# sec-bit/ckb-zkp

Measured on AMD Instinct MI355X. Metric: Groth16 proofs/sec (2^20 constraints, BN256), higher is better.
Workload: dtype u32 limbs (256-bit Montgomery integers); 1 GPU; Groth16 prove, MiMC-chain R1CS, 1048570 constraints (domain 2^20), 1258284 aux, bn254, G1 x4 + G2 x1 MSM + 4 NTT (7 in the reference: evaluation-form key); curve=bn254, log_domain=20, parallelism=independent proofs x1

## Files before the change

ckb_zkp_amd/csrc/msm.hip:

```cpp
#include <algorithm>
#include <cstdlib>
#include <cstring>
#include <map>
#include <type_traits>
#include <memory>
#include <mutex>
#include <vector>

#include "field_dev.hpp"
#include "internal.hpp"
#include "msm_digits.hpp"
#include "msm_small.hpp"
#include "msm_vtbl.hpp"

namespace zkp {

#if defined(ZKP_NO_SORT_PRIO)
#define ZKP_SORT_PRIO() do { } while (0)
#else
#define ZKP_SORT_PRIO() __builtin_amdgcn_s_setprio(3)
#endif

const MsmVtbl* msm_vtbl_c01();
const MsmVtbl* msm_vtbl_c02();
// ... 820 lines not shown
          constexpr int NT = decltype(nt)::value;
          hipLaunchKernelGGL((sort_hist_kernel<FrP, NT>), dim3(nblocks), dim3(NT), 0, st, sc, n, offset, scan_inf, mont, c, W, wide, nb_w,
                             LB, nbins1, hist, nblocks, tile, lgk);
        };
        if (nt_hist >= 1024) hist_l(std::integral_constant<int, 1024>{});
        else if (nt_hist >= 512) hist_l(std::integral_constant<int, 512>{});
        else hist_l(std::integral_constant<int, 256>{});
        exclusive_scan_u32(st, hist, offs, hist_n, ws.scan_tmp);
        if (staged_sub) {
          auto scat_l = [&](auto nt) {
            constexpr int NT = decltype(nt)::value;
            hipLaunchKernelGGL((sort_scatter_staged_kernel<FrP, NT>), dim3(nblocks), dim3(NT), staged_lds, st, sc, n, offset,
                               scan_inf, mont, be->n, c, W, wide, nb_w, LB, nbins1, offs, nblocks, tile, kv, lgk, grp, staged_sub);
          };
          if (nt_scat >= 1024) scat_l(std::integral_constant<int, 1024>{});
          else if (nt_scat >= 512) scat_l(std::integral_constant<int, 512>{});
          else scat_l(std::integral_constant<int, 256>{});
        } else {
          hipLaunchKernelGGL(sort_scatter_kernel<FrP>, dim3(nblocks), dim3(256), 0, st, sc, n, offset, scan_inf, mont, be->n, c, W, wide,
                             nb_w, LB, nbins1, offs, nblocks, tile, kv, lgk, grp);
        }
      };
      if (be->curve == ZKP_BN254) level1(Bn254Fr{});
      else level1(Bls381Fr{});
    }
    if (timed_scan) {
      ZKP_HIP(hipEventRecord(ctx->ev3, st));
      ZKP_HIP(hipEventSynchronize(ctx->ev3));
      ZKP_HIP(hipEventElapsedTime(ms_scan, ctx->ev2, ctx->ev3));
    }
    if (!reuse && !l1_reuse) ZKP_HIP(hipEventRecord(ws.l1_done, st));
    if (!reuse && !l1_reuse) ctx->mark(st, ":l1");
    if (!reuse)
      hipLaunchKernelGGL(sort_bin_kernel, dim3(nbins1), dim3(SORT_BIN_THREADS), ((size_t)4 << LB) + 4 * (size_t)SORT_BIN_STAGE, st,
                         kv, offs, nblocks, LB, vals, start, end, (l1_reuse || grp) ? be->filter_bit : -1);
    uint32_t* const sorted_vals = vals;
    const uint32_t max_tasks = nb + (uint32_t)(E / be->cap) + 1;
    uint32_t* sched = sw.sched.as<uint32_t>((size_t)2 * (nb + 2) + (size_t)8 * max_tasks + TM_WORDS + 8);
    uint32_t* tcount = sched;
    uint32_t* toff = tcount + (nb + 2);
    uint32_t* task_start = toff + (nb + 2);
    uint32_t* task_len = task_start + max_tasks;
    uint32_t* task_dst = task_len + max_tasks;
    uint32_t* long_list = task_dst + max_tasks;
    uint32_t* tmeta = long_list + max_tasks;
    uint4* desc = reinterpret_cast<uint4*>((reinterpret_cast<uintptr_t>(tmeta + TM_WORDS) + 15) & ~(uintptr_t)15);
    if (!reuse) {
      ZKP_HIP(hipMemsetAsync(tmeta, 0, TM_WORDS * 4, st));
      hipLaunchKernelGGL(task_count_kernel, dim3((nb + 256) / 256), dim3(256), 0, st, start, end, nb, tcount, be->cap);
      exclusive_scan_u32(st, tcount, toff, (size_t)nb + 1, ws.scan_tmp2);
      static const uint32_t tnt = [] { const char* e = getenv("ZKP_TASK_NT"); const int v = e ? atoi(e) : 1024; return (uint32_t)(v >= 1024 ? 1024 : v >= 512 ? 512 : 256); }();
      hipLaunchKernelGGL(task_fill_kernel, dim3((nb + tnt - 1) / tnt), dim3(tnt), 0, st, start, end, toff, nb, task_start,
                         task_len, task_dst, long_list, tmeta, be->cap);
      hipLaunchKernelGGL(task_cursor_kernel, dim3(1), dim3(64), 0, st, tmeta);
      hipLaunchKernelGGL(task_order_kernel, dim3((max_tasks + tnt - 1) / tnt), dim3(tnt), 0, st, task_start, task_len, task_dst,
                         toff + nb, tmeta, desc);
      ZKP_HIP(hipEventRecord(ws.sorted, st));
      ctx->mark(st, ":sorted");
    }
    MsmWorkspace& bws = bucket_ws >= 0 ? ctx->cur->ws[bucket_ws] : ws;
    char* buckets = reinterpret_cast<char*>(bws.buckets.get((size_t)2 * nb * XB + XB));
    char* task_partial = reinterpret_cast<char*>(ws.partial.get((size_t)max_tasks * XB));
    static const bool zero_all = getenv("ZKP_MEMSET_BUCKETS") && atoi(getenv("ZKP_MEMSET_BUCKETS")) != 0;
    const uint32_t init = into >= 0 ? 1u : 0u;
    if (init) {
      ZKP_REQUIRE(bws.chain_nb == nb && bws.chain_xb == XB, ZKP_ERR_BAD_ARG);
      ZKP_HIP(hipStreamWaitEvent(st, bws.acc_done, 0));
    } else if (zero_all) ZKP_HIP(hipMemsetAsync(buckets, 0, (size_t)nb * XB, st));
    else hipLaunchKernelGGL(zero_empty_buckets_kernel, dim3((nb + 255) / 256), dim3(256), 0, st, start, end, nb, buckets, (uint32_t)XB);
    bws.chain_nb = 0;
    const bool timed = ms_accumulate && ctx->profiling;
    if (timed) ZKP_HIP(hipEventRecord(ctx->ev2, st));
    static const uint32_t force_redo = getenv("ZKP_DEBUG_FORCE_REDO") && atoi(getenv("ZKP_DEBUG_FORCE_REDO")) != 0 ? 2u : 0u;
    ctx->mark(st, ":acc0");
    vt->accumulate(st, be->table, sorted_vals, desc, toff + nb, max_tasks, buckets, task_partial,
                   ws.redo.as<uint32_t>((size_t)max_tasks + 1), init | force_redo);
    ctx->mark(st, ":acc1");
    if (timed) {
      ZKP_HIP(hipEventRecord(ctx->ev3, st));
      ZKP_HIP(hipEventSynchronize(ctx->ev3));
      ZKP_HIP(hipEventElapsedTime(ms_accumulate, ctx->ev2, ctx->ev3));
    }
    static const int dbg = [] { const char* e = getenv("ZKP_DEBUG_MSM"); return e ? atoi(e) : 0; }();
    if (dbg) {
      uint32_t* rep = ws.redo.as<uint32_t>((size_t)max_tasks + 1);
      ZKP_HIP(hipStreamSynchronize(st));
      ZKP_HIP(hipMemsetAsync(rep, 0, 32, st));
      hipLaunchKernelGGL(sched_check_kernel, dim3(256), dim3(256), 0, st, toff, long_list, tmeta, nb, max_tasks, rep);
      uint32_t h[8];
      ZKP_HIP(hipMemcpyAsync(h, rep, 32, hipMemcpyDeviceToHost, st));
      ZKP_HIP(hipStreamSynchronize(st));
      printf("[msm] group=%d n=%zu nb=%u max_tasks=%u: toff inversions=%u max tasks/bucket=%u bad long_list=%u n_long=%u n_tasks=%u overflow=%u\n",
             be->group, n, nb, max_tasks, h[0], h[1], h[2], h[3], h[4], h[5]);
      fflush(stdout);
    }
#ifdef ZKP_ABLATION
    if (dbg != 2)
#endif
      vt->combine(st, long_list, tmeta + TM_NLONG, toff, task_partial, buckets, init);
    if (dbg) {
      hipError_t e = hipStreamSynchronize(st);
      printf("[msm] combine: %s\n", hipGetErrorString(e));
      fflush(stdout);
    }
    if (n_entries) {
      *n_entries = E;
      if (ctx->profiling) {
        uint32_t emitted = 0;
        ZKP_HIP(hipMemcpyAsync(&emitted, offs + hist_n - 1, 4, hipMemcpyDeviceToHost, st));
        ZKP_HIP(hipStreamSynchronize(st));
        *n_entries = emitted;
      }
    }
    if (var) {
      VarPlan& vp = var_plan(ctx, c, K, st);
      uint32_t lvl_off = 0, cnt = nb;
      for (int l = 0; l < c - 1; l++) {
        vt->pair(st, buckets + (size_t)lvl_off * XB, buckets + (size_t)(lvl_off + cnt) * XB, cnt / 2);
        lvl_off += cnt;
        cnt /= 2;
      }
      const char* roots = buckets + (size_t)lvl_off * XB;
      char* partial = reinterpret_cast<char*>(ws.tmp.get(((size_t)vp.n1 + 256 + 8) * XB));
      char* R = partial + (size_t)vp.n1 * XB;
      vt->segsum_desc(st, buckets, vp.d1.as<SegDesc>(vp.n1), vp.n1, partial);
      vt->segsum_desc(st, partial, vp.d2.as<SegDesc>(256), 256, R);
      vt->final_var(st, R, roots, c, K, (char*)out_dev_xyzz, out_jac);
      ZKP_HIP(hipGetLastError());
      if (out_xyz_host) {
        ZKP_HIP(hipMemcpyAsync(out_xyz_host, out_jac, jac_words * 4, hipMemcpyDeviceToHost, st));
        ZKP_HIP(hipStreamSynchronize(st));
      }
      return;
    }
    if (defer) {
      bws.chain_nb = nb;
      bws.chain_xb = XB;
      ZKP_HIP(hipEventRecord(bws.acc_done, st));
      vt->write_identity(st, (char*)out_dev_xyzz, out_jac);
      ZKP_HIP(hipGetLastError());
      ZKP_REQUIRE(!out_xyz_host, ZKP_ERR_BAD_ARG);
      return;
    }
#ifdef ZKP_ABLATION
    if (ctx->dbg_skip_k8) return;
#endif
    const int L = c - 1;
    SegPlan plan{};
    plan.L = L;
    const uint32_t chunk = ctx->batch_mode ? SEG_CHUNK_BATCH : SEG_CHUNK;
    plan.chunk = chunk;
    uint32_t lvl_off = 0, cnt = nb, blocks = 0;
    static const bool fuse_seg = !(getenv("ZKP_PAIR_TOP_FUSE_SEG") && atoi(getenv("ZKP_PAIR_TOP_FUSE_SEG")) == 0);
    int l_top = -1;
    char* top_base = nullptr;
    uint32_t top_cnt = 0;
    for (int l = 0; l < L; l++) {
      uint32_t next_off = lvl_off + cnt;
      static const bool top_fused = !(getenv("ZKP_PAIR_TOP") && atoi(getenv("ZKP_PAIR_TOP")) == 0);
      static const uint32_t top_max = [] {
        const char* e = getenv("ZKP_PAIR_TOP_MAX");
        uint32_t v = e ? (uint32_t)atoi(e) : PAIR_TOP_MAX;
        if (v < 2) v = PAIR_TOP_MAX;
        while (v & (v - 1)) v &= v - 1;
        return v;
      }();
      if (!top_fused || cnt > top_max) vt->pair(st, buckets + (size_t)lvl_off * XB, buckets + (size_t)next_off * XB, cnt / 2);
      else if (cnt == top_max || l == 0) {
        if (fuse_seg && cnt / 2 <= chunk) {
          l_top = l;
          top_base = buckets + (size_t)lvl_off * XB;
          top_cnt = cnt;
        } else {
          vt->pair_top(st, buckets + (size_t)lvl_off * XB, cnt);
        }
      }
      plan.first_block[l] = blocks;
      plan.off[l] = lvl_off + 1;
      plan.stride[l] = 2;
      plan.count[l] = cnt / 2;
      blocks += (cnt / 2 + chunk - 1) / chunk;
      lvl_off = next_off;
      cnt /= 2;
    }
    plan.first_block[L] = blocks;
    const char* root = buckets + (size_t)lvl_off * XB;
    char* partial = reinterpret_cast<char*>(ws.tmp.get(((size_t)blocks + 64) * XB));
    char* Obuf = partial + (size_t)blocks * XB;
    if (L > 0 && l_top >= 0) {
      SegPlan low = plan;
      low.L = l_top;
      const uint32_t blocks_low = plan.first_block[l_top];
      vt->pair_top_segsum(st, top_base, top_cnt, buckets, &low, partial, blocks_low);
      SegPlan p2{};
      p2.L = L;
      p2.chunk = chunk;
      for (int l = 0; l < L; l++) {
        p2.first_block[l] = l;
        if (l < l_top) {
          p2.off[l] = plan.first_block[l];
          p2.stride[l] = 1;
          p2.count[l] = plan.first_block[l + 1] - plan.first_block[l];
        } else {
          p2.off[l] = plan.off[l];
          p2.stride[l] = plan.stride[l];
          p2.count[l] = plan.count[l];
        }
        ZKP_REQUIRE(p2.count[l] <= chunk, ZKP_ERR_BAD_ARG);
      }
      p2.first_block[L] = L;
      vt->segsum(st, partial, &p2, Obuf, L, buckets, l_top);
    } else if (L > 0) {
      vt->segsum(st, buckets, &plan, partial, blocks, nullptr, 1 << 30);
      SegPlan p2{};
      p2.L = L;
      p2.chunk = chunk;
      for (int l = 0; l < L; l++) {
        p2.first_block[l] = l;
        p2.off[l] = plan.first_block[l];
        p2.stride[l] = 1;
        p2.count[l] = plan.first_block[l + 1] - plan.first_block[l];
        ZKP_REQUIRE(p2.count[l] <= chunk, ZKP_ERR_BAD_ARG);
      }
      p2.first_block[L] = L;
      vt->segsum(st, partial, &p2, Obuf, L, nullptr, 1 << 30);
    }
    vt->final(st, Obuf, L, root, (char*)out_dev_xyzz, out_jac);
    ctx->mark(st, ":reduced");
  }
  ZKP_HIP(hipGetLastError());
  if (out_xyz_host) {
    ZKP_HIP(hipMemcpyAsync(out_xyz_host, out_jac, jac_words * 4, hipMemcpyDeviceToHost, st));
    ZKP_HIP(hipStreamSynchronize(st));
  }
}

void msm_run_multi(zkp_ctx* ctx, size_t count, const uint64_t* handles, const size_t* offsets,
                   const uint64_t* const* scalars_dev, const size_t* ns, bool montgomery, uint64_t* out_xyz_host,
                   size_t slot_words) {
  if (count == 0) return;
  const size_t jw = slot_words;
  zkp_lane* L = ctx->cur;
  if (ctx->pinned_cap < count * jw * 4) {
    if (ctx->pinned) (void)hipHostFree(ctx->pinned);
    ctx->pinned = nullptr;
    ctx->pinned_cap = 0;
    ZKP_HIP(hipHostMalloc(reinterpret_cast<void**>(&ctx->pinned), count * jw * 4 + 4096));
    ctx->pinned_cap = count * jw * 4 + 4096;
  }
  constexpr int NW = zkp_lane::N_WS_MSM;
  const int NL = std::max(1, std::min(ctx->cfg.msm_batch_lanes, (int)zkp_ctx::N_LANES));
  auto stream_of = [&](int li, int w) { return w == 0 ? ctx->lanes[li].stream : ctx->lanes[li].ws[w].stream; };
  struct Restore {
    zkp_ctx* c;
    zkp_lane* cur;
    int idx;
    ~Restore() {
      c->cur = cur;
      c->cur_idx = idx;
    }
  } restore{ctx, ctx->cur, ctx->cur_idx};
  ZKP_HIP(hipEventRecord(L->ev_fork, L->stream));
  for (int li = 0; li < NL; li++)
    for (int w = 0; w < NW; w++)
      if (stream_of(li, w) != L->stream) ZKP_HIP(hipStreamWaitEvent(stream_of(li, w), L->ev_fork, 0));
  for (size_t k = 0; k < count; k++) {
    const int li = (int)((k / NW) % NL), w = (int)(k % NW);
    auto be = get_bases(ctx, handles[k]);
    const size_t words = 3 * (size_t)be->vt->fN;
    ZKP_REQUIRE(words <= jw, ZKP_ERR_BAD_ARG);
    ZKP_REQUIRE(offsets[k] <= be->n, ZKP_ERR_BAD_ARG);
    const size_t n = std::min(ns[k], be->n - offsets[k]);
    ctx->cur = &ctx->lanes[li];
    ctx->cur_idx = li;
    msm_run(ctx, handles[k], offsets[k], scalars_dev[k], n, montgomery, nullptr, nullptr, nullptr, nullptr, w);
    ZKP_HIP(hipMemcpyAsync(ctx->pinned + k * jw, ctx->lanes[li].ws[w].out.p, words * 4, hipMemcpyDeviceToHost, stream_of(li, w)));
  }
  ctx->cur = restore.cur;
  ctx->cur_idx = restore.idx;
  for (int li = 0; li < NL; li++)
    for (int w = 0; w < NW; w++) {
      if (stream_of(li, w) == L->stream) continue;
      ZKP_HIP(hipEventRecord(ctx->lanes[li].ws[w].done, stream_of(li, w)));
      ZKP_HIP(hipStreamWaitEvent(L->stream, ctx->lanes[li].ws[w].done, 0));
    }
  ZKP_HIP(hipStreamSynchronize(L->stream));
  memcpy(out_xyz_host, ctx->pinned, count * jw * 4);
}

void msm_run_batch(zkp_ctx* ctx, uint64_t handle, size_t count, const size_t* offsets, const uint64_t* const* scalars_dev,
                   const size_t* ns, bool montgomery, uint64_t* out_xyz_host) {
  if (count == 0) return;
  std::vector<uint64_t> handles(count, handle);
  msm_run_multi(ctx, count, handles.data(), offsets, scalars_dev, ns, montgomery, out_xyz_host,
                3 * (size_t)get_bases(ctx, handle)->vt->fN);
}

void msm_var_run(zkp_ctx* ctx, int curve, int group, const uint64_t* xy_host, const uint8_t* inf_host,
                 const uint64_t* scalars_host, size_t n, bool montgomery, uint64_t* out_xyz_host) {
  BasesEntry e;
  e.curve = curve;
  e.group = group;
  e.vt = msm_vtbl(curve, group);
  e.n = n;
  e.var = true;
  e.owns = false;
  e.c = n >= 4096 ? 16 : 8;
  if (const char* env = getenv("ZKP_MSM_VAR_C")) {
    int c = atoi(env);
    if (c == 4 || c == 8 || c == 16) e.c = c;
  }
  e.W = 256 / e.c;
  e.wide = e.W;
  while ((1 << e.lgk) < e.W) e.lgk++;
  ZKP_REQUIRE((double)n * e.W < 2147483000.0, ZKP_ERR_BAD_ARG);
  hipStream_t st = ctx->cur->stream;
  const size_t ab = e.vt->aff_bytes;
  uint64_t* sdev = nullptr;
  if (n) {
// ... 221 lines not shown
```

ckb_zkp_amd/csrc/msm_group.hip:

```cpp
#include "bucket_dev.hpp"
#include "coop_dev.hpp"
#include "ec_dev.hpp"
#include "glv.hpp"
#include "msm_vtbl.hpp"

#ifndef ZKP_CFG_CURVE
#error "compile with -DZKP_CFG_CURVE=0|1 -DZKP_CFG_GROUP=1|2"
#endif

namespace zkp {

#if ZKP_CFG_CURVE == 0
using CfgFq = Bn254Fq;
using CfgFr = Bn254Fr;
constexpr int CFG_BITS = 254;
#else
using CfgFq = Bls381Fq;
using CfgFr = Bls381Fr;
constexpr int CFG_BITS = 255;
#endif
#if ZKP_CFG_GROUP == 1
using CfgF = Fp<CfgFq>;
#else
using CfgF = Fp2<CfgFq>;
#endif
#define ZKP_CAT3(a, b, c) a##b##c
#define ZKP_SYM(name, cu, gr) ZKP_CAT3(name, cu, gr)
#define ZKP_CFG_SYM(name) ZKP_SYM(name##_c, ZKP_CFG_CURVE, ZKP_CFG_GROUP)

namespace ZKP_CFG_SYM(cfg) {}
using namespace ZKP_CFG_SYM(cfg);

template <class F>
__global__ void ingest_kernel(char* table, const uint8_t* inf, size_t n) {
  size_t i = (size_t)blockIdx.x * blockDim.x + threadIdx.x;
  if (i >= n) return;
  if (inf && inf[i]) Affine<F>::inf().store(table + i * Affine<F>::BYTES);
}

template <class F>
__global__ __launch_bounds__(128) void precompute_kernel(char* table, size_t n, int c, int W, int wide) {
  size_t i = (size_t)blockIdx.x * blockDim.x + threadIdx.x;
  if (i >= n) return;
  Affine<F> p = Affine<F>::load(table + i * Affine<F>::BYTES);
  XYZZ<F> acc = XYZZ<F>::from_affine(p);
  for (int w = 1; w < W; w++) {
    const int cw = w - 1 < wide ? c : c - 1;
    for (int k = 0; k < cw; k++) acc = acc.dbl();
    Affine<F> a = acc.to_affine();
    a.store(table + ((size_t)w * n + i) * Affine<F>::BYTES);
    acc = XYZZ<F>::from_affine(a);
  }
}

template <class F>
__global__ __launch_bounds__(256) void pair_kernel(const char* __restrict__ in, char* __restrict__ out,
                                                   uint32_t count) {
  __builtin_amdgcn_s_setprio(3);
  uint32_t k = blockIdx.x * blockDim.x + threadIdx.x;
  if (k >= count) return;
  BkPoint<F>::add_mem(in + (size_t)(2 * k) * BkPoint<F>::BYTES, in + (size_t)(2 * k + 1) * BkPoint<F>::BYTES,
                      out + (size_t)k * BkPoint<F>::BYTES);
}

constexpr int PAIR_TOP_THREADS = 512;
template <class F>
__device__ __forceinline__ void pair_top_body(char* __restrict__ base, uint32_t cnt) {
  char* in = base;
  for (; cnt > 1; cnt >>= 1) {
    char* out = in + (size_t)cnt * BkPoint<F>::BYTES;
    bool coop = false;
    if constexpr (QuadCoop<F>::ON) coop = cnt / 2 <= PAIR_TOP_THREADS / 4;
    if constexpr (QuadCoop<F>::ON) {
      if (coop) {
        const uint32_t k = threadIdx.x >> 2;
        if (k < cnt / 2)
          quad_add_any<F>(in + (size_t)(2 * k) * BkPoint<F>::BYTES, in + (size_t)(2 * k + 1) * BkPoint<F>::BYTES,
                          out + (size_t)k * BkPoint<F>::BYTES, threadIdx.x & 3);
      }
    }
    if (!coop)
      for (uint32_t k = threadIdx.x; k < cnt / 2; k += PAIR_TOP_THREADS)
        BkPoint<F>::add_mem(in + (size_t)(2 * k) * BkPoint<F>::BYTES, in + (size_t)(2 * k + 1) * BkPoint<F>::BYTES,
                            out + (size_t)k * BkPoint<F>::BYTES);
    __threadfence_block();
    __syncthreads();
    in = out;
  }
}
template <class F>
__global__ __launch_bounds__(PAIR_TOP_THREADS) void pair_top_kernel(char* __restrict__ base, uint32_t cnt) {
  __builtin_amdgcn_s_setprio(3);
  pair_top_body<F>(base, cnt);
}

template <class F>
__device__ __forceinline__ void segsum_body(const char* __restrict__ base, const SegPlan& plan, char* __restrict__ partial, uint32_t block,
                                            const char* __restrict__ base_hi, int l_hi) {
  extern __shared__ __attribute__((aligned(16))) char smem[];
  const uint32_t t = threadIdx.x;
  const bool act = t < 256;
  int l = 0;
  while (l + 1 < plan.L && block >= plan.first_block[l + 1]) l++;
  if (l >= l_hi) base = base_hi;
  uint32_t chunk = block - plan.first_block[l];
  uint32_t lo = chunk * plan.chunk;
  uint32_t hi = min(plan.count[l], lo + plan.chunk);
  if constexpr (BkPoint<F>::MEM_ADD) {
    char* my = smem + (act ? t : 0) * BkPoint<F>::BYTES;
    if (act) {
      BkPoint<F>::inf().store(my);
      for (uint32_t i = lo + t; i < hi; i += 256)
        BkPoint<F>::add_mem(my, base + ((size_t)plan.off[l] + (size_t)i * plan.stride[l]) * BkPoint<F>::BYTES, my);
    }
    __syncthreads();
    for (int s = 128; s > 0; s >>= 1) {
      bool coop = false;
      if constexpr (QuadCoop<F>::ON) {
        coop = s <= 64;
        if (coop && (int)(t >> 2) < s) {
          char* mine = smem + (t >> 2) * BkPoint<F>::BYTES;
          quad_add_any<F>(mine, smem + ((t >> 2) + s) * BkPoint<F>::BYTES, mine, t & 3);
        }
      }
      if (!coop && (int)t < s) BkPoint<F>::add_mem(my, smem + (t + s) * BkPoint<F>::BYTES, my);
      __syncthreads();
    }
    if (t == 0) BkPoint<F>::copy_point(partial + (size_t)block * BkPoint<F>::BYTES, my);
    return;
  }
  BkPoint<F> acc = BkPoint<F>::inf();
  if (act) {
    for (uint32_t i = lo + t; i < hi; i += 256)
      acc.add(BkPoint<F>::load(base + ((size_t)plan.off[l] + (size_t)i * plan.stride[l]) * BkPoint<F>::BYTES));
    acc.store(smem + t * BkPoint<F>::BYTES);
  }
  __syncthreads();
  for (int s = 128; s > 0; s >>= 1) {
    if ((int)t < s) {
      BkPoint<F> o = BkPoint<F>::load(smem + (t + s) * BkPoint<F>::BYTES);
      if (!o.is_inf() || !acc.is_inf()) {
        acc.add(o);
        acc.store(smem + t * BkPoint<F>::BYTES);
      }
    }
    __syncthreads();
  }
  if (t == 0) acc.store(partial + (size_t)block * BkPoint<F>::BYTES);
}
template <class F>
__global__ __launch_bounds__(256) void segsum_kernel(const char* __restrict__ base, SegPlan plan, char* __restrict__ partial,
                                                     const char* __restrict__ base_hi, int l_hi) {
  __builtin_amdgcn_s_setprio(3);
  segsum_body<F>(base, plan, partial, blockIdx.x, base_hi, l_hi);
}
template <class F>
__global__ __launch_bounds__(PAIR_TOP_THREADS) void pair_top_segsum_kernel(char* __restrict__ top_base, uint32_t top_cnt,
                                                                           const char* __restrict__ base, SegPlan plan,
                                                                           char* __restrict__ partial) {
  __builtin_amdgcn_s_setprio(3);
  if (blockIdx.x == 0) {
    pair_top_body<F>(top_base, top_cnt);
    return;
  }
  segsum_body<F>(base, plan, partial, blockIdx.x - 1, nullptr, 1 << 30);
}

constexpr uint32_t COMBINE_SMALL = 32;
template <class F>
__global__ __launch_bounds__(256) void combine_small_kernel(const uint32_t* __restrict__ long_list,
                                                            const uint32_t* __restrict__ n_long_dev,
                                                            const uint32_t* __restrict__ toff,
                                                            const char* __restrict__ partial,
                                                            char* __restrict__ buckets, uint32_t init) {
  __builtin_amdgcn_s_setprio(3);
  const uint32_t n_long = *n_long_dev;
  for (uint32_t w = blockIdx.x * blockDim.x + threadIdx.x; w < n_long; w += gridDim.x * blockDim.x) {
    const uint32_t b = long_list[w];
    const uint32_t p0 = toff[b], p1 = toff[b + 1];
    if (p1 - p0 > COMBINE_SMALL) continue;
    BkPoint<F> acc = BkPoint<F>::load(partial + (size_t)p0 * BkPoint<F>::BYTES);
    for (uint32_t i = p0 + 1; i < p1; i++) acc.add(BkPoint<F>::load(partial + (size_t)i * BkPoint<F>::BYTES));
    if (init) acc.add(BkPoint<F>::load(buckets + (size_t)b * BkPoint<F>::BYTES));
    acc.store(buckets + (size_t)b * BkPoint<F>::BYTES);
  }
}

template <class F>
__global__ __launch_bounds__(256) void combine_kernel(const uint32_t* __restrict__ long_list,
                                                      const uint32_t* __restrict__ n_long_dev,
                                                      const uint32_t* __restrict__ toff,
                                                      const char* __restrict__ partial, char* __restrict__ buckets, uint32_t init) {
  extern __shared__ __attribute__((aligned(16))) char smem[];
  const int lane = threadIdx.x & 63;
  const uint32_t wv = __builtin_amdgcn_readfirstlane(threadIdx.x >> 6), nw = blockDim.x >> 6;
  char* my = smem + (size_t)wv * 64 * BkPoint<F>::BYTES;
  const uint32_t n_long = *n_long_dev;
  for (uint32_t w = blockIdx.x * nw + wv; w < n_long; w += gridDim.x * nw) {
    const uint32_t b = __builtin_amdgcn_readfirstlane(long_list[w]);
    const uint32_t p0 = __builtin_amdgcn_readfirstlane(toff[b]), p1 = __builtin_amdgcn_readfirstlane(toff[b + 1]);
    if (p1 - p0 <= COMBINE_SMALL) continue;
    BkPoint<F> acc = BkPoint<F>::inf();
    for (uint32_t i = p0 + lane; i < p1; i += 64) acc.add(BkPoint<F>::load(partial + (size_t)i * BkPoint<F>::BYTES));
    acc.store(my + lane * BkPoint<F>::BYTES);
    __builtin_amdgcn_fence(__ATOMIC_RELEASE, "wavefront");
    for (int s = 32; s > 0; s >>= 1) {
      __builtin_amdgcn_wave_barrier();
      if (lane < s) {
        BkPoint<F> o = BkPoint<F>::load(my + (lane + s) * BkPoint<F>::BYTES);
        if (!o.is_inf()) {
          acc.add(o);
          acc.store(my + lane * BkPoint<F>::BYTES);
        }
      }
      __builtin_amdgcn_fence(__ATOMIC_ACQ_REL, "wavefront");
    }
    if (lane == 0) {
      if (init) acc.add(BkPoint<F>::load(buckets + (size_t)b * BkPoint<F>::BYTES));
      acc.store(buckets + (size_t)b * BkPoint<F>::BYTES);
    }
    __builtin_amdgcn_fence(__ATOMIC_ACQ_REL, "wavefront");
    __builtin_amdgcn_wave_barrier();
  }
}

template <class F>
__global__ __launch_bounds__(128) void final_kernel(const char* __restrict__ O, int L, const char* __restrict__ root,
                                                   char* __restrict__ out_xyzz, uint32_t* __restrict__ out_jac) {
  __builtin_amdgcn_s_setprio(3);
  extern __shared__ __attribute__((aligned(16))) char smem[];
  int t = threadIdx.x;
  if constexpr (QuadCoop<F>::ON && QuadCoop<F>::GROUP == 1) {
    const int q = t >> 2, role = t & 3;
    char* my = smem + q * BkPoint<F>::BYTES;
    if (role == 0) {
      if (q < L) BkPoint<F>::copy_point(my, O + (size_t)q * BkPoint<F>::BYTES);
      else if (q == L) BkPoint<F>::copy_point(my, root);
      else BkPoint<F>::inf().store(my);
    }
    __syncthreads();
    if (q < L)
      for (int k = 0; k < q; k++) quad_dbl_mem<typename QuadCoop<F>::P>(my, my, role);
    __syncthreads();
    for (int s = 16; s > 0; s >>= 1) {
      if (q < s) quad_add_mem<typename QuadCoop<F>::P>(my, smem + (q + s) * BkPoint<F>::BYTES, my, role);
      __syncthreads();
    }
    if (t == 0) {
      const XYZZ<F> res = BkPoint<F>::load(my).to_sat();
      if (out_xyzz) res.store(out_xyzz);
      if (out_jac) res.store_jacobian(out_jac);
    }
    return;
  }
  if constexpr (BkPoint<F>::MEM_ADD) {
    char* my = smem + t * BkPoint<F>::BYTES;
    if (t < L) BkPoint<F>::copy_point(my, O + (size_t)t * BkPoint<F>::BYTES);
    else if (t == L) BkPoint<F>::copy_point(my, root);
    else BkPoint<F>::inf().store(my);
    if (t < L && !BkPoint<F>::load(my).is_inf())
      for (int k = 0; k < t; k++) BkPoint<F>::dbl_mem(my, my);
    __syncthreads();
    for (int s = 32; s > 0; s >>= 1) {
      bool coop = false;
      if constexpr (QuadCoop<F>::ON) {
        coop = s <= 16;
        if (coop && (t >> 2) < s) {
          char* mine = smem + (t >> 2) * BkPoint<F>::BYTES;
          quad_add_any<F>(mine, smem + ((t >> 2) + s) * BkPoint<F>::BYTES, mine, t & 3);
        }
      }
      if (!coop && t < s) BkPoint<F>::add_mem(my, smem + (t + s) * BkPoint<F>::BYTES, my);
      __syncthreads();
    }
    if (t == 0) {
      const XYZZ<F> res = BkPoint<F>::load(my).to_sat();
      if (out_xyzz) res.store(out_xyzz);
      if (out_jac) res.store_jacobian(out_jac);
    }
    return;
  }
  BkPoint<F> acc = BkPoint<F>::inf();
  if (t < L) {
    acc = BkPoint<F>::load(O + (size_t)t * BkPoint<F>::BYTES);
    for (int k = 0; k < t; k++) acc = acc.dbl();
  } else if (t == L) {
    acc = BkPoint<F>::load(root);
  }
  acc.store(smem + t * BkPoint<F>::BYTES);
  __syncthreads();
  for (int s = 32; s > 0; s >>= 1) {
    if (t < s) {
      BkPoint<F> o = BkPoint<F>::load(smem + (t + s) * BkPoint<F>::BYTES);
      if (!o.is_inf() || !acc.is_inf()) {
        acc.add(o);
        acc.store(smem + t * BkPoint<F>::BYTES);
      }
    }
    __syncthreads();
  }
  if (t == 0) {
    const XYZZ<F> res = acc.to_sat();
    if (out_xyzz) res.store(out_xyzz);
    if (out_jac) res.store_jacobian(out_jac);
  }
}

template <class F>
__global__ __launch_bounds__(256) void segsum_desc_kernel(const char* __restrict__ base, const SegDesc* __restrict__ descs,
                                                          char* __restrict__ out) {
  __builtin_amdgcn_s_setprio(3);
  extern __shared__ __attribute__((aligned(16))) char smem[];
  const SegDesc d = descs[blockIdx.x];
  BkPoint<F> acc = BkPoint<F>::inf();
  for (uint32_t i = threadIdx.x; i < d.count; i += 256)
    acc.add(BkPoint<F>::load(base + ((size_t)d.off + (size_t)i * d.stride) * BkPoint<F>::BYTES));
  acc.store(smem + threadIdx.x * BkPoint<F>::BYTES);
  __syncthreads();
// ... 413 lines not shown
  }
  XYZZ<F> r = L_inf[m] ? XYZZ<F>::inf() : XYZZ<F>::from_affine(Affine<F>::load(L_xy + m * Affine<F>::BYTES));
  r.add(acc.neg());
  r.to_affine().store(out_xy + m * Affine<F>::BYTES);
  out_inf[m] = r.is_inf() ? 1 : 0;
}
#endif

namespace ZKP_CFG_SYM(cfg) {
#if ZKP_CFG_GROUP == 1
template <class F>
__device__ __forceinline__ void jac_dbl(F& X, F& Y, F& Z) {
  F A = X.sqr(), B = Y.sqr();
  F C = B.sqr();
  F D = ((X + B).sqr() - A - C).dbl();
  F E = A.dbl() + A;
  F Fq = E.sqr();
  F Z3 = (Y * Z).dbl();
  X = Fq - D.dbl();
  Y = E * (D - X) - C.dbl().dbl().dbl();
  Z = Z3;
}
__global__ __launch_bounds__(128) void assemble_g1_part1_kernel(char* __restrict__ res, size_t slot,
                                                                const uint32_t* __restrict__ rs,
                                                                uint32_t* __restrict__ out,
                                                                uint32_t* __restrict__ flags) {
  using F = CfgF;
  using G = GlvConst<CfgFq>;
  __builtin_amdgcn_s_setprio(3);
  extern __shared__ __attribute__((aligned(16))) char smem[];
  constexpr int NB = G::BITS;
  constexpr size_t JB = 3 * 4 * F::N;
  const int t = threadIdx.x, chain = t >> 6, lane = t & 63;
  char* D = smem + (size_t)chain * NB * JB;
  char* red = smem + 2 * NB * JB + (size_t)chain * 64 * XYZZ<F>::BYTES;
  Fp<CfgFr> k = Fp<CfgFr>::load(rs + (chain == 0 ? 8 : 0)).from_mont();
  uint32_t k1[5], k2[5];
  int neg1, neg2;
  glv_decompose<G>(k.v, k1, &neg1, k2, &neg2);
  if (lane == 0) {
    XYZZ<F> p = XYZZ<F>::load(res + (size_t)chain * slot);
    F X, Y, Z;
    if (out) {
      Affine<F> a = p.to_affine();
      if (chain == 0) {
        a.store(out);
        flags[0] = p.is_inf() ? 1 : 0;
      }
      X = a.x, Y = a.y, Z = p.is_inf() ? F::zero() : F::one();
    } else {
      X = p.x * p.zz.sqr();
      Y = p.y * p.zzz.sqr();
      Z = p.is_inf() ? F::zero() : p.zzz;
    }
    for (int b = 0; b < NB; b++) {
      X.store(D + (size_t)b * JB);
      Y.store(D + (size_t)b * JB + 4 * F::N);
      Z.store(D + (size_t)b * JB + 8 * F::N);
      if (b + 1 < NB) jac_dbl(X, Y, Z);
    }
  }
  __syncthreads();
  F beta;
#pragma unroll
  for (int i = 0; i < F::N; i++) beta.v[i] = G::BETA_MONT[i];
  XYZZ<F> acc = XYZZ<F>::inf();
  for (int b = lane; b < NB; b += 64) {
    const bool t1 = (k1[b >> 5] >> (b & 31)) & 1, t2 = (k2[b >> 5] >> (b & 31)) & 1;
    if (!(t1 || t2)) continue;
    const F X = F::load(D + (size_t)b * JB), Y = F::load(D + (size_t)b * JB + 4 * F::N), Z = F::load(D + (size_t)b * JB + 8 * F::N);
    if (Z.is_zero()) continue;
    const F zz = Z.sqr();
    const F zzz = zz * Z;
    if (t1) acc.add(XYZZ<F>{X, neg1 ? Y.neg() : Y, zz, zzz});
    if (t2) acc.add(XYZZ<F>{beta * X, neg2 ? Y.neg() : Y, zz, zzz});
  }
  acc.store(red + (size_t)lane * XYZZ<F>::BYTES);
  __syncthreads();
  for (int s2 = 32; s2 > 0; s2 >>= 1) {
    if (lane < s2) {
      XYZZ<F> o = XYZZ<F>::load(red + (size_t)(lane + s2) * XYZZ<F>::BYTES);
      if (!o.is_inf() || !acc.is_inf()) {
        acc.add(o);
        acc.store(red + (size_t)lane * XYZZ<F>::BYTES);
      }
    }
    __syncthreads();
  }
  if (t == 0) {
    acc.add(XYZZ<F>::load(smem + 2 * NB * JB + 64 * XYZZ<F>::BYTES));
    acc.store(res + 5 * slot);
  }
}
__global__ __launch_bounds__(64) void assemble_g1_part2_kernel(char* __restrict__ res, size_t slot,
                                                               uint32_t* __restrict__ out,
                                                               uint32_t* __restrict__ flags, int c_off_words) {
  using F = CfgF;
  if (threadIdx.x || blockIdx.x) return;
  XYZZ<F> acc = XYZZ<F>::load(res + 5 * slot);
  acc.add(XYZZ<F>::load(res + 3 * slot));
  acc.add(XYZZ<F>::load(res + 4 * slot));
  if (!out) {
    acc.store(res + 5 * slot);
    return;
  }
  Affine<F> c = acc.to_affine();
  c.store(out + c_off_words);
  flags[2] = acc.is_inf() ? 1 : 0;
}
#else
__global__ __launch_bounds__(64) void assemble_g2_kernel(const char* __restrict__ res, size_t slot,
                                                         uint32_t* __restrict__ out, uint32_t* __restrict__ flags,
                                                         int out_off_words) {
  if (threadIdx.x || blockIdx.x) return;
  XYZZ<CfgF> p = XYZZ<CfgF>::load(res + 2 * slot);
  p.to_affine().store(out + out_off_words);
  flags[1] = p.is_inf() ? 1 : 0;
}
#endif
}

void ZKP_CFG_SYM(msm_accumulate_launch)(hipStream_t, const char*, const uint32_t*, const uint4*, const uint32_t*, uint32_t,
                                        char*, char*, uint32_t*, uint32_t);

namespace {
using F = CfgF;
constexpr size_t XB = XYZZ<F>::BYTES;
constexpr size_t BB = BkPoint<F>::BYTES;
void l_ingest(hipStream_t s, char* table, const uint8_t* inf, size_t n) {
  hipLaunchKernelGGL(ingest_kernel<F>, dim3((n + 255) / 256), dim3(256), 0, s, table, inf, n);
}
void l_precompute(hipStream_t s, char* table, size_t n, int c, int W, int wide) {
  hipLaunchKernelGGL(precompute_kernel<F>, dim3((n + 127) / 128), dim3(128), 0, s, table, n, c, W, wide);
}
void l_combine(hipStream_t s, const uint32_t* long_list, const uint32_t* n_long_dev, const uint32_t* toff,
               const char* partial, char* buckets, uint32_t init) {
  hipLaunchKernelGGL(combine_small_kernel<F>, dim3(256), dim3(256), 0, s, long_list, n_long_dev, toff, partial, buckets, init);
  hipLaunchKernelGGL(combine_kernel<F>, dim3(512), dim3(256), 256 * BB, s, long_list, n_long_dev, toff, partial, buckets, init);
}
void l_pair(hipStream_t s, const char* in, char* out, uint32_t count) {
  hipLaunchKernelGGL(pair_kernel<F>, dim3((count + 255) / 256), dim3(256), 0, s, in, out, count);
}
void l_pair_top(hipStream_t s, char* base, uint32_t count) {
  hipLaunchKernelGGL(pair_top_kernel<F>, dim3(1), dim3(PAIR_TOP_THREADS), 0, s, base, count);
}
void l_segsum(hipStream_t s, const char* base, const SegPlan* plan, char* partial, uint32_t blocks, const char* base_hi, int l_hi) {
  hipLaunchKernelGGL(segsum_kernel<F>, dim3(blocks), dim3(256), 256 * BB, s, base, *plan, partial, base_hi, l_hi);
}
void l_pair_top_segsum(hipStream_t s, char* top_base, uint32_t top_cnt, const char* base, const SegPlan* plan, char* partial,
                       uint32_t blocks) {
  hipLaunchKernelGGL(pair_top_segsum_kernel<F>, dim3(1 + blocks), dim3(PAIR_TOP_THREADS), 256 * BB, s, top_base, top_cnt, base, *plan,
                     partial);
}
void l_final(hipStream_t s, const char* O, int L, const char* root, char* out_xyzz, uint32_t* out_jac) {
  constexpr int threads = (QuadCoop<F>::ON && QuadCoop<F>::GROUP == 1) ? 128 : 64;
  hipLaunchKernelGGL(final_kernel<F>, dim3(1), dim3(threads), 64 * BB, s, O, L, root, out_xyzz, out_jac);
}
void l_identity(hipStream_t s, char* out_xyzz, uint32_t* out_jac) {
  hipLaunchKernelGGL(write_identity_kernel<F>, dim3(1), dim3(64), 0, s, out_xyzz, out_jac);
}
void l_fold(hipStream_t s, const uint32_t* pts, int k, uint32_t* out_jac) {
  hipLaunchKernelGGL(fold_kernel<F>, dim3(1), dim3(64), 0, s, pts, k, out_jac);
}
void l_segsum_desc(hipStream_t s, const char* base, const SegDesc* descs, uint32_t n_desc, char* out) {
  if (n_desc) hipLaunchKernelGGL(segsum_desc_kernel<F>, dim3(n_desc), dim3(256), 256 * BB, s, base, descs, out);
}
void l_final_var(hipStream_t s, const char* R, const char* roots, int c, int W, char* out_xyzz, uint32_t* out_jac) {
  hipLaunchKernelGGL(final_var_kernel<F>, dim3(1), dim3(256), 256 * BB, s, R, roots, c, W, out_xyzz, out_jac);
}
#if ZKP_CFG_GROUP == 1
void l_gfft(hipStream_t s, const char* xy, const uint8_t* inf, size_t n_in, const uint32_t* scal, const uint32_t* tw, uint32_t log_n,
            char* X, char* out_xy, uint8_t* out_inf) {
  const size_t N = (size_t)1 << log_n;
  hipLaunchKernelGGL((gfft_scale_kernel<F, CFG_BITS>), dim3((N + 127) / 128), dim3(128), 0, s, xy, inf, n_in, scal, log_n, X);
  for (uint32_t st = 1; st <= log_n; st++)
    hipLaunchKernelGGL((gfft_stage_kernel<F, CFG_BITS>), dim3((N / 2 + 127) / 128), dim3(128), 0, s, X, tw, log_n, st);
  hipLaunchKernelGGL(gfft_affine_kernel<F>, dim3((N + 127) / 128), dim3(128), 0, s, X, N, out_xy, out_inf);
}
void l_lfold(hipStream_t s, const char* L_xy, const uint8_t* L_inf, size_t n_vars, const uint32_t* col_ptr, const uint32_t* rows,
             const uint8_t* kind, const uint32_t* coeff, const char* G_xy, const uint8_t* G_inf, char* out_xy, uint8_t* out_inf) {
  if (n_vars)
    hipLaunchKernelGGL((lfold_kernel<F, CFG_BITS>), dim3((n_vars + 127) / 128), dim3(128), 0, s, L_xy, L_inf, n_vars, col_ptr, rows,
                       kind, coeff, G_xy, G_inf, out_xy, out_inf);
}
#endif
void l_fold_slots(hipStream_t s, const char* gathered, size_t rank_stride, int world, size_t slot, uint32_t mask,
                  char* res) {
  hipLaunchKernelGGL(fold_slots_kernel<F>, dim3(1), dim3(64), 0, s, gathered, rank_stride, world, slot, mask, res);
}
void l_into_affine(hipStream_t s, const uint32_t* jac, uint32_t* xy, uint32_t* inf) {
  hipLaunchKernelGGL(into_affine_kernel<F>, dim3(1), dim3(64), 0, s, jac, xy, inf);
}
void l_fold_affine_batch(hipStream_t s, const uint32_t* ja, const uint32_t* jb, const uint32_t* has_b, int k, uint32_t* xy,
                         uint32_t* inf) {
  if (k > 0) hipLaunchKernelGGL(fold_affine_batch_kernel<F>, dim3((k + 63) / 64), dim3(64), 0, s, ja, jb, has_b, k, xy, inf);
}
void l_decompress(hipStream_t s, const uint32_t* bytes, size_t n, const uint32_t* bcoef, char* xy, uint8_t* inf, uint32_t* status) {
  hipLaunchKernelGGL(curve_b_kernel<F>, dim3(1), dim3(64), 0, s, const_cast<uint32_t*>(bcoef));
  if (n) hipLaunchKernelGGL(decompress_kernel<F>, dim3((n + 63) / 64), dim3(64), 0, s, bytes, n, bcoef, xy, inf, status);
}
void l_compress(hipStream_t s, const char* xy, const uint8_t* inf, size_t n, uint32_t* bytes) {
  if (n) hipLaunchKernelGGL(compress_kernel<F>, dim3((n + 63) / 64), dim3(64), 0, s, xy, inf, n, bytes);
}
void l_subgroup_check(hipStream_t s, const char* xy, const uint8_t* inf, size_t n, const uint32_t* bcoef, uint32_t* status) {
  hipLaunchKernelGGL(curve_b_kernel<F>, dim3(1), dim3(64), 0, s, const_cast<uint32_t*>(bcoef));
  if (n) hipLaunchKernelGGL(subgroup_check_kernel<F>, dim3((n + 63) / 64), dim3(64), 0, s, xy, inf, n, bcoef, status);
}
void l_from_jacobian(hipStream_t s, const uint32_t* jac, char* out) {
  hipLaunchKernelGGL(from_jacobian_kernel<F>, dim3(1), dim3(64), 0, s, jac, out);
}
void l_fixed_base(hipStream_t s, const uint32_t* base, const uint32_t* scalars, size_t n, char* out_xy,
                  uint8_t* out_inf) {
  hipLaunchKernelGGL((fixed_base_kernel<F, CFG_BITS>), dim3((n + 127) / 128), dim3(128), 0, s, base, scalars, n,
                     out_xy, out_inf);
}
#if ZKP_CFG_GROUP == 1
void l_assemble_g1_p1(hipStream_t s, char* res, size_t slot, const uint32_t* rs, uint32_t* out, uint32_t* flags) {
  const size_t lds = 2 * (size_t)GlvConst<CfgFq>::BITS * 3 * 4 * F::N + 2 * 64 * XB;
  hipLaunchKernelGGL(assemble_g1_part1_kernel, dim3(1), dim3(128), lds, s, res, slot, rs, out, flags);
}
void l_assemble_g1_p2(hipStream_t s, char* res, size_t slot, uint32_t* out, uint32_t* flags, int c_off_words) {
  hipLaunchKernelGGL(assemble_g1_part2_kernel, dim3(1), dim3(64), 0, s, res, slot, out, flags, c_off_words);
}
#else
void l_assemble_g2(hipStream_t s, const char* res, size_t slot, uint32_t* out, uint32_t* flags, int off) {
  hipLaunchKernelGGL(assemble_g2_kernel, dim3(1), dim3(64), 0, s, res, slot, out, flags, off);
}
#endif
}

const MsmVtbl* ZKP_CFG_SYM(msm_vtbl)() {
  static const MsmVtbl v = {
      F::N, Affine<F>::BYTES, XYZZ<F>::BYTES, BkPoint<F>::BYTES, CFG_BITS,
      l_ingest, l_precompute, ZKP_CFG_SYM(msm_accumulate_launch), l_combine, l_pair, l_segsum, l_final, l_identity, l_fold,
      l_into_affine, l_fold_affine_batch, l_decompress, l_compress, l_subgroup_check, l_from_jacobian, l_fixed_base, l_segsum_desc, l_final_var, l_fold_slots,
#if ZKP_CFG_GROUP == 1
      l_assemble_g1_p1, l_assemble_g1_p2, nullptr,
#else
      nullptr, nullptr, l_assemble_g2,
#endif
      l_pair_top,
#if ZKP_CFG_GROUP == 1
      l_gfft, l_lfold,
#else
      nullptr, nullptr,
#endif
      l_pair_top_segsum,
  };
  return &v;
}

}
```

ckb_zkp_amd/csrc/msm_vtbl.hpp:

```cpp
#pragma once
#include <hip/hip_runtime.h>
#include <stddef.h>
#include <stdint.h>

namespace zkp {

constexpr int SEG_CHUNK = 1024;
constexpr int SEG_CHUNK_BATCH = 4096;
constexpr uint32_t MSM_TASK_CAP = 128;
struct SegPlan {
  int L;
  uint32_t chunk;
  uint32_t first_block[26];
  uint32_t off[25];
  uint32_t stride[25];
  uint32_t count[25];
};

struct SegDesc {
  uint32_t off, stride, count, out;
};

struct MsmVtbl {
  int fN;
  size_t aff_bytes, xyzz_bytes;
  size_t bucket_bytes;
  int scalar_bits;
  void (*ingest)(hipStream_t, char* table, const uint8_t* inf, size_t n);
  void (*precompute)(hipStream_t, char* table, size_t n, int c, int W, int wide);
  void (*accumulate)(hipStream_t, const char* table, const uint32_t* vals, const uint4* desc,
                     const uint32_t* n_tasks_dev, uint32_t max_tasks, char* buckets, char* partial, uint32_t* redo, uint32_t init);
  void (*combine)(hipStream_t, const uint32_t* long_list, const uint32_t* n_long_dev, const uint32_t* toff,
                  const char* partial, char* buckets, uint32_t init);
  void (*pair)(hipStream_t, const char* in, char* out, uint32_t count);
  void (*segsum)(hipStream_t, const char* base, const SegPlan* plan, char* partial, uint32_t blocks, const char* base_hi, int l_hi);
  void (*final)(hipStream_t, const char* O, int L, const char* root, char* out_xyzz, uint32_t* out_jac);
  void (*write_identity)(hipStream_t, char* out_xyzz, uint32_t* out_jac);
  void (*fold)(hipStream_t, const uint32_t* pts, int k, uint32_t* out_jac);
  void (*into_affine)(hipStream_t, const uint32_t* jac, uint32_t* xy, uint32_t* inf);
  void (*fold_affine_batch)(hipStream_t, const uint32_t* jac_a, const uint32_t* jac_b, const uint32_t* has_b, int k,
                            uint32_t* xy, uint32_t* inf);
  void (*decompress)(hipStream_t, const uint32_t* bytes, size_t n, const uint32_t* bcoef, char* xy, uint8_t* inf, uint32_t* status);
  void (*compress)(hipStream_t, const char* xy, const uint8_t* inf, size_t n, uint32_t* bytes);
  void (*subgroup_check)(hipStream_t, const char* xy, const uint8_t* inf, size_t n, const uint32_t* bcoef, uint32_t* status);
  void (*from_jacobian)(hipStream_t, const uint32_t* jac, char* out_xyzz);
  void (*fixed_base)(hipStream_t, const uint32_t* base, const uint32_t* scalars, size_t n, char* out_xy,
                     uint8_t* out_inf);
  void (*segsum_desc)(hipStream_t, const char* base, const SegDesc* descs, uint32_t n_desc, char* out);
  void (*final_var)(hipStream_t, const char* R, const char* roots, int c, int W, char* out_xyzz, uint32_t* out_jac);
  void (*fold_slots)(hipStream_t, const char* gathered, size_t rank_stride, int world, size_t slot, uint32_t mask,
                     char* res);
  void (*assemble_g1_part1)(hipStream_t, char* res, size_t slot, const uint32_t* rs, uint32_t* out, uint32_t* flags);
  void (*assemble_g1_part2)(hipStream_t, char* res, size_t slot, uint32_t* out, uint32_t* flags, int c_off_words);
  void (*assemble_g2)(hipStream_t, const char* res, size_t slot, uint32_t* out, uint32_t* flags, int out_off_words);
  void (*pair_top)(hipStream_t, char* base, uint32_t count);
  void (*gfft)(hipStream_t, const char* xy, const uint8_t* inf, size_t n_in, const uint32_t* scal, const uint32_t* tw, uint32_t log_n,
               char* X, char* out_xy, uint8_t* out_inf);
  void (*lfold)(hipStream_t, const char* L_xy, const uint8_t* L_inf, size_t n_vars, const uint32_t* col_ptr, const uint32_t* rows,
                const uint8_t* kind, const uint32_t* coeff, const char* G_xy, const uint8_t* G_inf, char* out_xy, uint8_t* out_inf);
  void (*pair_top_segsum)(hipStream_t, char* top_base, uint32_t top_cnt, const char* base, const SegPlan* plan, char* partial,
                          uint32_t blocks);
};
constexpr uint32_t PAIR_TOP_MAX = 2048;

const MsmVtbl* msm_vtbl(int curve, int group);

}
```

Before: 144.7 proofs/s.

## Reduce MSM bucket tree in LDS-resident blocks instead of per-level pair kernels

Adds a reduce_block kernel that loads a contiguous block of 2^K buckets into shared memory and performs several pairwise-reduction levels in place. It emits the per-level odd-slot partials needed for the weighted bucket sum and writes the block roots. The host then rebuilds the segment-sum plan so those partials feed pair_top_segsum and a second segsum pass. This replaces one global-memory pair kernel per level with a few LDS-resident passes, cutting global traffic and launch count. In exchange it adds a complex index mapping, an extra segsum stage and a large LDS footprint per block, which may limit occupancy.

```diff
diff --git a/ckb_zkp_amd/csrc/msm.hip b/ckb_zkp_amd/csrc/msm.hip
--- a/ckb_zkp_amd/csrc/msm.hip
+++ b/ckb_zkp_amd/csrc/msm.hip
@@ -996,19 +996,88 @@
     plan.chunk = chunk;
     uint32_t lvl_off = 0, cnt = nb, blocks = 0;
     static const bool fuse_seg = !(getenv("ZKP_PAIR_TOP_FUSE_SEG") && atoi(getenv("ZKP_PAIR_TOP_FUSE_SEG")) == 0);
+    static const bool top_fused = !(getenv("ZKP_PAIR_TOP") && atoi(getenv("ZKP_PAIR_TOP")) == 0);
+    static const uint32_t top_max = [] {
+      const char* e = getenv("ZKP_PAIR_TOP_MAX");
+      uint32_t v = e ? (uint32_t)atoi(e) : PAIR_TOP_MAX;
+      if (v < 2) v = PAIR_TOP_MAX;
+      while (v & (v - 1)) v &= v - 1;
+      return v;
+    }();
+    const int RK = vt->reduce_block_k, RS = vt->reduce_block_s;
+    if (L > 0 && fuse_seg && top_fused && top_max >= (1u << RK) && top_max / 2 <= chunk && nb >= (1u << RK)) {
+      struct Pass {
+        uint32_t in_off, out_off, nblk, poff;
+      } pass[8];
+      int npass = 0, l = 0;
+      SegPlan low{};
+      low.chunk = SEG_CHUNK_BLOCKS;
+      uint32_t poff = 0, lb = 0;
+      while (cnt >= (1u << RK) && (npass == 0 || cnt > top_max)) {
+        ZKP_REQUIRE(npass < 8, ZKP_ERR_BAD_ARG);
+        const uint32_t nblk = cnt >> RK, nout = cnt >> RS;
+        uint32_t out_off = lvl_off;
+        for (int j = 0; j < RS; j++, l++) {
+          low.first_block[l] = lb;
+          low.off[l] = poff + (uint32_t)j * nout;
+          low.stride[l] = 1;
+          low.count[l] = nout;
+          lb += (nout + low.chunk - 1) / low.chunk;
+          out_off += cnt >> j;
+        }
+        pass[npass++] = {lvl_off, out_off, nblk, poff};
+        poff += (uint32_t)RS * nout;
+        lvl_off = out_off;
+        cnt = nout;
+      }
+      const int l_blk = l;
+      low.L = l_blk;
+      low.first_block[l_blk] = lb;
+      char* top = buckets + (size_t)lvl_off * XB;
+      const uint32_t top_n = cnt;
+      SegPlan p2{};
+      p2.L = L;
+      p2.chunk = chunk;
+      for (l = 0; l < L; l++) {
+        p2.first_block[l] = l;
+        if (l < l_blk) {
+          p2.off[l] = low.first_block[l];
+          p2.stride[l] = 1;
+          p2.count[l] = low.first_block[l + 1] - low.first_block[l];
+        } else {
+          p2.off[l] = lvl_off + 1;
+          p2.stride[l] = 2;
+          p2.count[l] = cnt / 2;
+          lvl_off += cnt;
+          cnt /= 2;
+        }
+        ZKP_REQUIRE(p2.count[l] <= chunk, ZKP_ERR_BAD_ARG);
+      }
+      p2.first_block[L] = L;
+      ZKP_REQUIRE(cnt == 1, ZKP_ERR_BAD_ARG);
+      const char* root = buckets + (size_t)lvl_off * XB;
+      char* partial = reinterpret_cast<char*>(ws.tmp.get(((size_t)poff + lb + 64) * XB));
+      char* partial2 = partial + (size_t)poff * XB;
+      char* Obuf = partial2 + (size_t)lb * XB;
+      for (int i = 0; i < npass; i++)
+        vt->reduce_block(st, buckets + (size_t)pass[i].in_off * XB, buckets + (size_t)pass[i].out_off * XB,
+                         partial + (size_t)pass[i].poff * XB, pass[i].nblk);
+      vt->pair_top_segsum(st, top, top_n, partial, &low, partial2, lb);
+      vt->segsum(st, partial2, &p2, Obuf, L, buckets, l_blk);
+      vt->final(st, Obuf, L, root, (char*)out_dev_xyzz, out_jac);
+      ctx->mark(st, ":reduced");
+      ZKP_HIP(hipGetLastError());
+      if (out_xyz_host) {
+        ZKP_HIP(hipMemcpyAsync(out_xyz_host, out_jac, jac_words * 4, hipMemcpyDeviceToHost, st));
+        ZKP_HIP(hipStreamSynchronize(st));
+      }
+      return;
+    }
     int l_top = -1;
     char* top_base = nullptr;
     uint32_t top_cnt = 0;
     for (int l = 0; l < L; l++) {
       uint32_t next_off = lvl_off + cnt;
-      static const bool top_fused = !(getenv("ZKP_PAIR_TOP") && atoi(getenv("ZKP_PAIR_TOP")) == 0);
-      static const uint32_t top_max = [] {
-        const char* e = getenv("ZKP_PAIR_TOP_MAX");
-        uint32_t v = e ? (uint32_t)atoi(e) : PAIR_TOP_MAX;
-        if (v < 2) v = PAIR_TOP_MAX;
-        while (v & (v - 1)) v &= v - 1;
-        return v;
-      }();
       if (!top_fused || cnt > top_max) vt->pair(st, buckets + (size_t)lvl_off * XB, buckets + (size_t)next_off * XB, cnt / 2);
       else if (cnt == top_max || l == 0) {
         if (fuse_seg && cnt / 2 <= chunk) {
diff --git a/ckb_zkp_amd/csrc/msm_group.hip b/ckb_zkp_amd/csrc/msm_group.hip
--- a/ckb_zkp_amd/csrc/msm_group.hip
+++ b/ckb_zkp_amd/csrc/msm_group.hip
@@ -164,6 +164,83 @@
     return;
   }
   segsum_body<F>(base, plan, partial, blockIdx.x - 1, nullptr, 1 << 30);
+}
+
+#ifndef ZKP_RB_LDS_CAP
+#define ZKP_RB_LDS_CAP (80 * 1024)
+#endif
+#ifndef ZKP_RB_STEPS
+#define ZKP_RB_STEPS 99
+#endif
+template <class F>
+struct ReduceBlock {
+  static constexpr int pick_k() {
+    int k = 1;
+    while (((size_t)BkPoint<F>::BYTES << (k + 1)) <= ZKP_RB_LDS_CAP) k++;
+    return k;
+  }
+  static constexpr int K = pick_k();
+  static constexpr int S = ZKP_RB_STEPS < K ? ZKP_RB_STEPS : K;
+  static constexpr int R = 1 << (K - S);
+  static constexpr int THREADS = 1 << (K - 1);
+  static constexpr int LDS_BYTES = BkPoint<F>::BYTES << K;
+  static_assert(2 * LDS_BYTES <= 160 * 1024 && BkPoint<F>::BYTES % 16 == 0 && THREADS >= 64, "block does not fit");
+};
+template <class F>
+__global__ __launch_bounds__(ReduceBlock<F>::THREADS) void reduce_block_kernel(const char* __restrict__ in, char* __restrict__ roots,
+                                                                               char* __restrict__ partial, uint32_t nblk) {
+  using RB = ReduceBlock<F>;
+  constexpr int K = RB::K, S = RB::S, R = RB::R, T = RB::THREADS;
+  constexpr uint32_t PB = BkPoint<F>::BYTES;
+  __shared__ __attribute__((aligned(16))) char blk[RB::LDS_BYTES];
+#ifndef ZKP_RB_NO_PRIO
+  __builtin_amdgcn_s_setprio(3);
+#endif
+  const uint32_t t = threadIdx.x, b = blockIdx.x;
+  {
+    const uint4* src = reinterpret_cast<const uint4*>(in + (size_t)b * RB::LDS_BYTES);
+    uint4* dst = reinterpret_cast<uint4*>(blk);
+    for (uint32_t i = t; i < RB::LDS_BYTES / 16; i += T) dst[i] = src[i];
+  }
+  __syncthreads();
+#pragma unroll 1
+  for (int s = 0; s < S; s++) {
+    const int w = K - s - 1;
+    const uint32_t n_add = (uint32_t)(s + 1) << w;
+    bool coop = false;
+#ifndef ZKP_RB_NO_QUAD
+    if constexpr (QuadCoop<F>::ON) coop = n_add <= T / 4;
+#endif
+    const uint32_t a = coop ? t >> 2 : t;
+    if (a < n_add) {
+      const uint32_t g = a >> w, i = a & ((1u << w) - 1);
+      uint32_t sa, sb;
+      if (g == (uint32_t)s) {
+        sa = (2 * i) << s;
+        sb = (2 * i + 1) << s;
+      } else {
+        const int ts = s - (int)g - 1;
+        const uint32_t e = i << (ts + 1);
+        sa = (2 * e + 1) << g;
+        sb = (2 * (e + (1u << ts)) + 1) << g;
+      }
+      char* pa = blk + sa * PB;
+      const char* pb = blk + sb * PB;
+      if constexpr (QuadCoop<F>::ON) {
+        if (coop) quad_add_any<F>(pa, pb, pa, t & 3);
+      }
+      if (!coop) BkPoint<F>::add_mem(pa, pb, pa);
+    }
+    __syncthreads();
+  }
+  constexpr uint32_t PW = PB / 4;
+  const uint32_t* lw = reinterpret_cast<const uint32_t*>(blk);
+  for (uint32_t i = t; i < (S + 1) * R * PW; i += T) {
+    const uint32_t q = i / PW, wd = i % PW, p = q / R, e = q % R;
+    const uint32_t slot = p < (uint32_t)S ? (2 * (e << (S - p - 1)) + 1) << p : e << S;
+    char* o = p < (uint32_t)S ? partial + (((size_t)p * nblk + b) * R + e) * PB : roots + ((size_t)b * R + e) * PB;
+    reinterpret_cast<uint32_t*>(o)[wd] = lw[slot * PW + wd];
+  }
 }
 
 constexpr uint32_t COMBINE_SMALL = 32;
@@ -883,6 +960,9 @@
   hipLaunchKernelGGL(pair_top_segsum_kernel<F>, dim3(1 + blocks), dim3(PAIR_TOP_THREADS), 256 * BB, s, top_base, top_cnt, base, *plan,
                      partial);
 }
+void l_reduce_block(hipStream_t s, const char* in, char* roots, char* partial, uint32_t nblk) {
+  hipLaunchKernelGGL(reduce_block_kernel<F>, dim3(nblk), dim3(ReduceBlock<F>::THREADS), 0, s, in, roots, partial, nblk);
+}
 void l_final(hipStream_t s, const char* O, int L, const char* root, char* out_xyzz, uint32_t* out_jac) {
   constexpr int threads = (QuadCoop<F>::ON && QuadCoop<F>::GROUP == 1) ? 128 : 64;
   hipLaunchKernelGGL(final_kernel<F>, dim3(1), dim3(threads), 64 * BB, s, O, L, root, out_xyzz, out_jac);
@@ -977,6 +1057,7 @@
       nullptr, nullptr,
 #endif
       l_pair_top_segsum,
+      ReduceBlock<F>::K, ReduceBlock<F>::S, l_reduce_block,
   };
   return &v;
 }
diff --git a/ckb_zkp_amd/csrc/msm_vtbl.hpp b/ckb_zkp_amd/csrc/msm_vtbl.hpp
--- a/ckb_zkp_amd/csrc/msm_vtbl.hpp
+++ b/ckb_zkp_amd/csrc/msm_vtbl.hpp
@@ -60,7 +60,10 @@
                 const uint8_t* kind, const uint32_t* coeff, const char* G_xy, const uint8_t* G_inf, char* out_xy, uint8_t* out_inf);
   void (*pair_top_segsum)(hipStream_t, char* top_base, uint32_t top_cnt, const char* base, const SegPlan* plan, char* partial,
                           uint32_t blocks);
+  int reduce_block_k, reduce_block_s;
+  void (*reduce_block)(hipStream_t, const char* in, char* roots, char* partial, uint32_t nblk);
 };
+constexpr uint32_t SEG_CHUNK_BLOCKS = 512;
 constexpr uint32_t PAIR_TOP_MAX = 2048;
 
 const MsmVtbl* msm_vtbl(int curve, int group);
```

Measured after the change: 136.0 proofs/s. -6.0%, worse.
